# google-research/big_vision

Hardware: NVIDIA H100
Metric: siglip_vit_b16_pairs_per_sec (higher is better)
Workload: dtype bf16

## Files before the change

big_vision_b200/csrc/api.cu:

```cuda
#include "../../include/bv_b200.h"

#include "host_utils.h"
#include "kernels.h"

using namespace bv;

static inline cudaStream_t S(void* s) { return reinterpret_cast<cudaStream_t>(s); }

extern "C" {

const char* bv_last_error_string(void) { return last_error(); }
int bv_version(void) { return 100; }

int bv_device_supported(void) {
  int dev = 0;
  if (cudaGetDevice(&dev) != cudaSuccess) return 0;
  int major = 0;
  if (cudaDeviceGetAttribute(&major, cudaDevAttrComputeCapabilityMajor, dev) != cudaSuccess) return 0;
  return major == 9 ? 1 : 0;
}

int bv_gemm(const bv_gemm_args* a, void* stream) {
  if (!a) { set_error("bv_gemm: null args"); return BV_ERR_INVALID; }
  GemmArgs g;
  g.A = a->A; g.B = a->B; g.D = a->D; g.D2 = a->D2; g.bias = a->bias; g.aux = a->aux;
  g.colsum = a->colsum;
  g.M = a->M; g.N = a->N; g.K = a->K;
  g.lda = a->lda; g.ldb = a->ldb; g.ldd = a->ldd; g.ldd2 = a->ldd2; g.ldaux = a->ldaux;
  g.a_mn = a->a_mn; g.b_mn = a->b_mn; g.epi = a->epilogue; g.out_dtype = a->out_dtype;
  g.reduce_out = a->reduce_out; g.splits = a->splits; g.block_n = a->block_n;
  g.aux_row_mod = a->aux_row_mod; g.alpha = a->alpha;
  return launch_gemm(g, S(stream));
}

int bv_layernorm_fwd(const void* x, int x_dtype, const float* scale, const float* bias, void* y,
                     int y_dtype, float* mean, float* rstd, int64_t rows, int32_t d, float eps,
                     void* stream) {
  return launch_layernorm_fwd(x, x_dtype, scale, bias, y, y_dtype, mean, rstd, rows, d, eps, S(stream));
}
int bv_layernorm_bwd(const void* dy, int dy_dtype, const void* x, int x_dtype, const float* scale,
                     const float* mean, const float* rstd, const void* dres, void* dx,
                     int dx_dtype, float* dscale, float* dbias, float* dx_colsum, int64_t rows,
                     int32_t d, void* stream) {
  return launch_layernorm_bwd(dy, dy_dtype, x, x_dtype, scale, mean, rstd, dres, dx, dx_dtype,
                              dscale, dbias, dx_colsum, rows, d, S(stream));
}

static AttnArgs to_attn(const bv_attn_args& a) {
  AttnArgs r;
  r.q = a.q; r.k = a.k; r.v = a.v; r.o = a.o; r.lse = a.lse;
  r.B = a.B; r.H = a.H; r.Nq = a.Nq; r.Nk = a.Nk;
  r.ldq = a.ldq; r.ldk = a.ldk; r.ldv = a.ldv; r.ldo = a.ldo;
  r.bsq = a.bsq; r.bsk = a.bsk; r.bsv = a.bsv; r.bso = a.bso;
  r.scale = a.scale;
  return r;
}
int bv_attention_fwd(const bv_attn_args* a, void* stream) { return bv_attention_fwd_hd(a, 64, stream); }
int bv_attention_fwd_hd(const bv_attn_args* a, int32_t head_dim, void* stream) {
  if (!a) { set_error("bv_attention_fwd: null args"); return BV_ERR_INVALID; }
  return launch_attention_fwd(to_attn(*a), head_dim, S(stream));
}
int bv_attention_bwd(const bv_attn_bwd_args* a, void* stream) { return bv_attention_bwd_hd(a, 64, stream); }
int bv_attention_bwd_hd(const bv_attn_bwd_args* a, int32_t head_dim, void* stream) {
  if (!a) { set_error("bv_attention_bwd: null args"); return BV_ERR_INVALID; }
  AttnBwdArgs g;
  g.f = to_attn(a->fwd);
  g.d_o = a->d_o; g.lddo = a->lddo; g.bsdo = a->bsdo;
  g.dq = a->dq; g.dk = a->dk; g.dv = a->dv;
  g.lddq = a->lddq; g.lddk = a->lddk; g.lddv = a->lddv;
  g.bsdq = a->bsdq; g.bsdk = a->bsdk; g.bsdv = a->bsdv;
  g.dq_colsum = a->dq_colsum; g.dk_colsum = a->dk_colsum; g.dv_colsum = a->dv_colsum;
  g.delta = a->delta; g.dq_accum = a->dq_accum;
  return launch_attention_bwd(g, head_dim, S(stream));
}

int bv_patchify(const float* image, void* patches, int64_t n, int32_t H, int32_t W, int32_t C,
                int32_t P, void* stream) {
  return launch_patchify(image, patches, n, H, W, C, P, S(stream));
}
int bv_patchify_u8(const uint8_t* image, void* patches, int64_t n, int32_t H, int32_t W, int32_t C,
                   int32_t P, float vmin, float vmax, float in_min, float in_max, int32_t clip_values,
                   void* stream) {
  return launch_patchify_u8(image, patches, n, H, W, C, P, vmin, vmax, in_min, in_max, clip_values, S(stream));
}
int bv_embed_fwd(const int32_t* ids, const float* table, const float* pos, void* out,
                 int out_dtype, int64_t n, int32_t L, int32_t d, int32_t vocab, void* stream) {
  return launch_embed_fwd(ids, table, pos, out, out_dtype, n, L, d, vocab, S(stream));
}
int bv_embed_bwd(const int32_t* ids, const void* dy, int dy_dtype, float* dtable, float* dpos,
                 int64_t n, int32_t L, int32_t d, int32_t vocab, void* stream) {
  return launch_embed_bwd(ids, dy, dy_dtype, dtable, dpos, n, L, d, vocab, S(stream));
}
int bv_colsum(const void* x, int x_dtype, float* out, int64_t rows, int64_t cols, int64_t ld,
              void* stream) {
  return launch_colsum(x, x_dtype, out, rows, cols, ld, S(stream));
}
int bv_cast(const void* src, int src_dtype, void* dst, int dst_dtype, int64_t n, void* stream) {
  return launch_cast(src, src_dtype, dst, dst_dtype, n, S(stream));
}
int bv_l2norm_fwd(const void* x, int x_dtype, float* z, float* norm, int64_t n, int32_t d,
                  float eps, void* stream) {
  return launch_l2norm_fwd(x, x_dtype, z, norm, n, d, eps, S(stream));
}
int bv_l2norm_bwd(const float* dz, const float* z, const float* norm, void* dx, int dx_dtype,
                  int64_t n, int32_t d, float eps, void* stream) {
  return launch_l2norm_bwd(dz, z, norm, dx, dx_dtype, n, d, eps, S(stream));
}
int bv_pool_fwd(const void* x, int x_dtype, void* y, int y_dtype, int64_t n, int32_t N, int32_t d,
                int32_t mode, int32_t tok, void* stream) {
  return launch_pool(x, x_dtype, y, y_dtype, n, N, d, mode, tok, S(stream));
}
int bv_pool_bwd(const void* dy, int dy_dtype, void* dx, int dx_dtype, int64_t n, int32_t N,
                int32_t d, int32_t mode, int32_t tok, void* stream) {
  return launch_pool_bwd(dy, dy_dtype, dx, dx_dtype, n, N, d, mode, tok, S(stream));
}
int bv_pool_max_bwd(const void* dy, int dy_dtype, const void* x, int x_dtype, void* dx, int dx_dtype,
                    int64_t n, int32_t N, int32_t d, void* stream) {
  return launch_pool_max_bwd(dy, dy_dtype, x, x_dtype, dx, dx_dtype, n, N, d, S(stream));
}
int bv_broadcast_row(const void* x, int x_dtype, const float* row, void* y, int y_dtype,
                     int64_t rows, int32_t d, void* stream) {
  return launch_add_rows(x, x_dtype, row, y, y_dtype, rows, d, S(stream));
}
int bv_tanh_fwd(const void* x, void* y, int dtype, int64_t n, void* stream) {
  return launch_tanh_fwd(x, y, dtype, n, S(stream));
// ... 107 lines not shown
```

big_vision_b200/csrc/attention.cu:

```cuda
#include "common.cuh"
#include "host_utils.h"
#include "kernels.h"

namespace bv {

namespace {

constexpr int T = 64;
constexpr int BOX_BYTES = T * 64 * 2;
constexpr float LOG2E = 1.4426950408889634f;
constexpr float LN2 = 0.6931471805599453f;
constexpr int THREADS = 128;

template <int DH>
struct Geo {
  static_assert(DH == 64 || DH == 72 || DH == 80 || DH == 96 || DH == 104, "head dims 64, 72, 80, 96, 104");
  static constexpr int TILE_BYTES = DH > 64 ? 2 * BOX_BYTES : BOX_BYTES;
  static constexpr int KSTEPS = (DH + 15) / 16;
  static_assert(KSTEPS >= 4 && KSTEPS <= 8, "one or two 64-column boxes");
  static constexpr int R = DH / 2;
  static constexpr int FWD_SMEM = 5 * TILE_BYTES + 1024 + 64;
  static constexpr int BWD_SMEM = 6 * TILE_BYTES + BOX_BYTES + 1024 + 64;
};

__device__ __forceinline__ float ex2(float x) {
  float y;
  asm("ex2.approx.ftz.f32 %0, %1;" : "=f"(y) : "f"(x));
  return y;
}

int make_tmap_bnd(CUtensorMap* m, const void* ptr, int dh, int H, int64_t N, int64_t B, int64_t ld, int64_t bs) {
  if (dh == 64) {
    uint64_t dims[3] = {static_cast<uint64_t>(H) * 64, static_cast<uint64_t>(N), static_cast<uint64_t>(B)};
    uint64_t strides[2] = {static_cast<uint64_t>(ld) * 2, static_cast<uint64_t>(bs) * 2};
    uint32_t box[3] = {64, T, 1};
    return make_tmap(m, CU_TENSOR_MAP_DATA_TYPE_BFLOAT16, 3, ptr, dims, strides, box, true);
  }
  uint64_t dims[4] = {static_cast<uint64_t>(dh), static_cast<uint64_t>(H), static_cast<uint64_t>(N),
                      static_cast<uint64_t>(B)};
  uint64_t strides[3] = {static_cast<uint64_t>(dh) * 2, static_cast<uint64_t>(ld) * 2, static_cast<uint64_t>(bs) * 2};
  uint32_t box[4] = {64, 1, T, 1};
  return make_tmap(m, CU_TENSOR_MAP_DATA_TYPE_BFLOAT16, 4, ptr, dims, strides, box, true);
}

template <int DH>
__device__ __forceinline__ void load_tile(uint32_t dst, const CUtensorMap* m, uint32_t bar, int h, int row, int b) {
  if constexpr (DH == 64) {
    tma_load_3d(dst, m, bar, h * DH, row, b);
  } else {
    tma_load_4d(dst, m, bar, 0, h, row, b);
    tma_load_4d(dst + BOX_BYTES, m, bar, 64, h, row, b);
  }
}

__device__ __forceinline__ uint64_t desc_k(uint32_t tile) { return wgmma_desc_sw128(tile, 16u, 1024u); }
__device__ __forceinline__ uint64_t desc_mn(uint32_t tile) { return wgmma_desc_sw128(tile, 8192u, 1024u); }
constexpr uint64_t KSTEP_K = 32 >> 4, KSTEP_MN = 2048 >> 4;

template <int TA, int TB, int R>
__device__ __forceinline__ void wgmma_ss_dh(float (&d)[R], uint64_t a, uint64_t b, int scale_d) {
  if constexpr (R == 32) wgmma_ss_n64<TA, TB>(d, a, b, scale_d);
  else if constexpr (R == 36) wgmma_ss_n72<TA, TB>(d, a, b, scale_d);
  else if constexpr (R == 40) wgmma_ss_n80<TA, TB>(d, a, b, scale_d);
  else if constexpr (R == 48) wgmma_ss_n96<TA, TB>(d, a, b, scale_d);
  else wgmma_ss_n104<TA, TB>(d, a, b, scale_d);
}
template <int TB, int R>
__device__ __forceinline__ void wgmma_rs_dh(float (&d)[R], const uint32_t (&a)[4], uint64_t b, int scale_d) {
  if constexpr (R == 32) wgmma_rs_n64<TB>(d, a, b, scale_d);
  else if constexpr (R == 36) wgmma_rs_n72<TB>(d, a, b, scale_d);
  else if constexpr (R == 40) wgmma_rs_n80<TB>(d, a, b, scale_d);
  else if constexpr (R == 48) wgmma_rs_n96<TB>(d, a, b, scale_d);
  else wgmma_rs_n104<TB>(d, a, b, scale_d);
}

template <int DH>
__device__ __forceinline__ void mma_tile_kk(float (&d)[32], uint32_t a_tile, uint32_t b_tile) {
  const uint64_t a = desc_k(a_tile), b = desc_k(b_tile);
#pragma unroll
  for (int k = 0; k < 4; ++k) wgmma_ss_n64<0, 0>(d, a + k * KSTEP_K, b + k * KSTEP_K, k > 0 ? 1 : 0);
  if constexpr (DH > 64) {
    const uint64_t a1 = desc_k(a_tile + BOX_BYTES), b1 = desc_k(b_tile + BOX_BYTES);
#pragma unroll
    for (int k = 0; k < Geo<DH>::KSTEPS - 4; ++k) wgmma_ss_n64<0, 0>(d, a1 + k * KSTEP_K, b1 + k * KSTEP_K, 1);
  }
}
template <int R>
__device__ __forceinline__ void mma_tile_rs(float (&d)[R], const uint32_t (&p)[4][4], uint32_t b_tile) {
  const uint64_t b = desc_mn(b_tile);
#pragma unroll
  for (int k = 0; k < 4; ++k) wgmma_rs_dh<1>(d, p[k], b + k * KSTEP_MN, 1);
}

__device__ __forceinline__ void to_frags(const float (&s)[32], uint32_t (&p)[4][4]) {
#pragma unroll
  for (int kk = 0; kk < 4; ++kk) {
    p[kk][0] = pack_bf16(s[8 * kk + 0], s[8 * kk + 1]);
    p[kk][1] = pack_bf16(s[8 * kk + 2], s[8 * kk + 3]);
    p[kk][2] = pack_bf16(s[8 * kk + 4], s[8 * kk + 5]);
    p[kk][3] = pack_bf16(s[8 * kk + 6], s[8 * kk + 7]);
  }
}

template <int R>
__device__ __forceinline__ void zero(float (&d)[R]) {
#pragma unroll
  for (int i = 0; i < R; ++i) d[i] = 0.f;
}

struct FwdDev {
  int H, Nq, Nk, QT, NB;
  float scale_log2;
  float* lse;
  bf16* o;
  long long ldo, bso;
};

template <int DH>
__global__ void __launch_bounds__(THREADS)
// ... 48 lines not shown
      const int key = kbase + 8 * (i >> 2) + (i & 1);
      s[i] = key < p.Nk ? s[i] * p.scale_log2 : -INFINITY;
      mx[(i >> 1) & 1] = fmaxf(mx[(i >> 1) & 1], s[i]);
    }
    float corr[2];
#pragma unroll
    for (int r = 0; r < 2; ++r) {
      mx[r] = fmaxf(mx[r], __shfl_xor_sync(0xffffffffu, mx[r], 1));
      mx[r] = fmaxf(mx[r], __shfl_xor_sync(0xffffffffu, mx[r], 2));
      corr[r] = ex2(m[r] - mx[r]);
      m[r] = mx[r];
      l[r] *= corr[r];
    }
#pragma unroll
    for (int i = 0; i < 32; ++i) {
      const int r = (i >> 1) & 1;
      s[i] = ex2(s[i] - m[r]);
      l[r] += s[i];
      o[i] *= corr[r];
    }
#pragma unroll
    for (int i = 32; i < G::R; ++i) o[i] *= corr[(i >> 1) & 1];
    uint32_t pf[4][4];
    to_frags(s, pf);
    wgmma_fence_regs(o);
    wgmma_fence();
    mma_tile_rs(o, pf, v_s + slot * TILE_BYTES);
    wgmma_commit();
    wgmma_wait<0>();
    wgmma_fence_regs(o);
    __syncthreads();
    if (tid == 0 && j + 2 < p.NB) load_kv(j + 2);
  }
#pragma unroll
  for (int r = 0; r < 2; ++r) {
    l[r] += __shfl_xor_sync(0xffffffffu, l[r], 1);
    l[r] += __shfl_xor_sync(0xffffffffu, l[r], 2);
  }
  const float inv[2] = {1.f / l[0], 1.f / l[1]};
#pragma unroll
  for (int r = 0; r < 2; ++r) {
    const int q = qt * T + 16 * warp + (lane >> 2) + 8 * r;
    if (q >= p.Nq) continue;
    bf16* orow = p.o + b * p.bso + static_cast<long long>(q) * p.ldo + h * DH + 2 * (lane & 3);
#pragma unroll
    for (int jj = 0; jj < DH / 8; ++jj)
      *reinterpret_cast<uint32_t*>(orow + 8 * jj) = pack_bf16(o[4 * jj + 2 * r] * inv[r], o[4 * jj + 2 * r + 1] * inv[r]);
    if ((lane & 3) == 0) p.lse[(static_cast<long long>(b) * p.H + h) * p.Nq + q] = (m[r] + __log2f(l[r])) * LN2;
  }
}

struct BwdDev {
  int H, Nq, Nk, QT, KT;
  long long B;
  float scale, scale_log2;
  const float* lse;
  const float* delta;
  float* dq_accum;
  bf16* dk; bf16* dv;
  long long lddk, bsdk, lddv, bsdv;
  float* dk_colsum; float* dv_colsum;
};

template <int R>
__device__ __forceinline__ void tile_colsum(const float (&d)[R], float mul, int row0, int nvalid, float* colsum,
                                            int lane) {
#pragma unroll
  for (int jj = 0; jj < R / 4; ++jj) {
    float c[2] = {0.f, 0.f};
#pragma unroll
    for (int r = 0; r < 2; ++r) {
      if (row0 + 8 * r >= nvalid) continue;
      c[0] += round_bf16(d[4 * jj + 2 * r] * mul);
      c[1] += round_bf16(d[4 * jj + 2 * r + 1] * mul);
    }
#pragma unroll
    for (int e = 0; e < 2; ++e) {
      c[e] += __shfl_xor_sync(0xffffffffu, c[e], 4);
      c[e] += __shfl_xor_sync(0xffffffffu, c[e], 8);
      c[e] += __shfl_xor_sync(0xffffffffu, c[e], 16);
    }
    if (lane < 4) {
      atomicAdd(colsum + 8 * jj + 2 * lane, c[0]);
      atomicAdd(colsum + 8 * jj + 2 * lane + 1, c[1]);
    }
  }
}

template <int DH>
__global__ void __launch_bounds__(THREADS)
attn_bwd_kernel(const __grid_constant__ CUtensorMap tmQ, const __grid_constant__ CUtensorMap tmK,
                const __grid_constant__ CUtensorMap tmV, const __grid_constant__ CUtensorMap tmdO, const BwdDev p) {
  using G = Geo<DH>;
  constexpr int TILE_BYTES = G::TILE_BYTES;
  extern __shared__ uint8_t smem_raw[];
  const uint32_t k_s = (smem_u32(smem_raw) + 1023u) & ~1023u, v_s = k_s + TILE_BYTES, q_s = k_s + 2 * TILE_BYTES,
                 do_s = k_s + 4 * TILE_BYTES, ds_s = k_s + 6 * TILE_BYTES;
  const uint32_t kv_bar = ds_s + BOX_BYTES;
  auto q_bar = [&](int s) { return kv_bar + 8u * (1 + s); };

  const int kt = static_cast<int>(blockIdx.x % p.KT);
  const int bh = static_cast<int>(blockIdx.x / p.KT);
  const int h = bh % p.H, b = bh / p.H;
  const int tid = threadIdx.x, lane = tid & 31, warp = tid >> 5;

  auto load_q = [&](int i) {
    const int s = i & 1;
    mbar_expect_tx(q_bar(s), 2 * TILE_BYTES);
    load_tile<DH>(q_s + s * TILE_BYTES, &tmQ, q_bar(s), h, i * T, b);
    load_tile<DH>(do_s + s * TILE_BYTES, &tmdO, q_bar(s), h, i * T, b);
  };
  if (tid == 0) {
    mbar_init(kv_bar, 1);
    mbar_init(q_bar(0), 1);
    mbar_init(q_bar(1), 1);
    fence_barrier_init();
    mbar_expect_tx(kv_bar, 2 * TILE_BYTES);
    load_tile<DH>(k_s, &tmK, kv_bar, h, kt * T, b);
    load_tile<DH>(v_s, &tmV, kv_bar, h, kt * T, b);
    load_q(0);
    if (p.QT > 1) load_q(1);
  }
  __syncthreads();

  float dk[G::R], dv[G::R];
  zero(dk);
  zero(dv);
  const long long bhq = (static_cast<long long>(b) * p.H + h) * p.Nq;
  const int cols = p.H * DH;
  const int key_row = 16 * warp + (lane >> 2);
  mbar_wait(kv_bar, 0);
  for (int i = 0; i < p.QT; ++i) {
    const int slot = i & 1;
    mbar_wait(q_bar(slot), (i >> 1) & 1);
    const uint32_t qi = q_s + slot * TILE_BYTES, doi = do_s + slot * TILE_BYTES;
    float st[32], dpt[32];
    wgmma_fence();
    mma_tile_kk<DH>(st, k_s, qi);
    mma_tile_kk<DH>(dpt, v_s, doi);
    wgmma_commit();
    float lse2[16], dl[16];
#pragma unroll
    for (int c = 0; c < 16; ++c) {
      const int q = i * T + 8 * (c >> 1) + 2 * (lane & 3) + (c & 1);
      lse2[c] = q < p.Nq ? p.lse[bhq + q] * LOG2E : INFINITY;
      dl[c] = q < p.Nq ? p.delta[bhq + q] : 0.f;
    }
    wgmma_wait<0>();
    wgmma_fence_regs(st);
    wgmma_fence_regs(dpt);
#pragma unroll
    for (int e = 0; e < 32; ++e) {
      const int c = 2 * (e >> 2) + (e & 1);
      st[e] = ex2(st[e] * p.scale_log2 - lse2[c]);
      dpt[e] = st[e] * (dpt[e] - dl[c]);
    }
    uint32_t pf[4][4], sf[4][4];
    to_frags(st, pf);
    to_frags(dpt, sf);
#pragma unroll
    for (int kk = 0; kk < 4; ++kk) {
#pragma unroll
      for (int f = 0; f < 4; ++f) {
        const int r = key_row + 8 * (f & 1);
        const int chunk = 2 * kk + (f >> 1);
        const uint32_t addr = ds_s + r * 128 + ((chunk ^ (r & 7)) << 4) + 4 * (lane & 3);
        asm volatile("st.shared.b32 [%0], %1;" ::"r"(addr), "r"(sf[kk][f]) : "memory");
      }
    }
    fence_proxy_async();
    __syncthreads();
    float dq[G::R];
    wgmma_fence_regs(dv);
    wgmma_fence_regs(dk);
    wgmma_fence();
    mma_tile_rs(dv, pf, doi);
    mma_tile_rs(dk, sf, qi);
    {
      const uint64_t a = desc_mn(ds_s), bk = desc_mn(k_s);
#pragma unroll
      for (int k = 0; k < 4; ++k) wgmma_ss_dh<1, 1>(dq, a + k * KSTEP_MN, bk + k * KSTEP_MN, k > 0 ? 1 : 0);
    }
    wgmma_commit();
    wgmma_wait<0>();
    wgmma_fence_regs(dv);
    wgmma_fence_regs(dk);
    wgmma_fence_regs(dq);
#pragma unroll
    for (int r = 0; r < 2; ++r) {
      const int q = i * T + 16 * warp + (lane >> 2) + 8 * r;
      if (q >= p.Nq) continue;
      float* dst = p.dq_accum + ((static_cast<long long>(kt) * p.B + b) * p.Nq + q) * cols + h * DH + 2 * (lane & 3);
#pragma unroll
      for (int jj = 0; jj < DH / 8; ++jj)
        *reinterpret_cast<float2*>(dst + 8 * jj) = make_float2(dq[4 * jj + 2 * r] * p.scale,
                                                               dq[4 * jj + 2 * r + 1] * p.scale);
    }
    __syncthreads();
    if (tid == 0 && i + 2 < p.QT) load_q(i + 2);
  }
  const int k0 = kt * T + key_row;
#pragma unroll
  for (int r = 0; r < 2; ++r) {
    const int key = k0 + 8 * r;
    if (key >= p.Nk) continue;
    bf16* kr = p.dk + b * p.bsdk + static_cast<long long>(key) * p.lddk + h * DH + 2 * (lane & 3);
    bf16* vr = p.dv + b * p.bsdv + static_cast<long long>(key) * p.lddv + h * DH + 2 * (lane & 3);
#pragma unroll
    for (int jj = 0; jj < DH / 8; ++jj) {
      *reinterpret_cast<uint32_t*>(kr + 8 * jj) = pack_bf16(dk[4 * jj + 2 * r] * p.scale, dk[4 * jj + 2 * r + 1] * p.scale);
      *reinterpret_cast<uint32_t*>(vr + 8 * jj) = pack_bf16(dv[4 * jj + 2 * r], dv[4 * jj + 2 * r + 1]);
    }
  }
  if (p.dk_colsum != nullptr) tile_colsum(dk, p.scale, k0, p.Nk, p.dk_colsum + h * DH, lane);
  if (p.dv_colsum != nullptr) tile_colsum(dv, 1.f, k0, p.Nk, p.dv_colsum + h * DH, lane);
}

template <int DH>
__global__ void __launch_bounds__(256)
attn_delta_kernel(const bf16* __restrict__ o, const bf16* __restrict__ d_o, float* __restrict__ delta,
                  int64_t B, int H, int N, int64_t ldo, int64_t bso, int64_t lddo, int64_t bsdo) {
  constexpr int LOG2_LANES = DH == 64 ? 3 : 4, LANES = 1 << LOG2_LANES;
  const int64_t total = B * N * H;
  const int chunk = threadIdx.x & (LANES - 1);
  for (int64_t r = (blockIdx.x * static_cast<int64_t>(blockDim.x) + threadIdx.x) >> LOG2_LANES; r < total;
       r += (static_cast<int64_t>(gridDim.x) * blockDim.x) >> LOG2_LANES) {
    const int h = static_cast<int>(r % H);
    const int64_t bt = r / H;
    const int t = static_cast<int>(bt % N);
    const int64_t b = bt / N;
    float acc = 0.f;
    if (chunk < DH / 8) {
      const uint4 ao = ld_nc_na(reinterpret_cast<const uint4*>(o + b * bso + t * ldo + h * DH + chunk * 8));
      const uint4 ad = ld_nc_na(reinterpret_cast<const uint4*>(d_o + b * bsdo + t * lddo + h * DH + chunk * 8));
      acc = bf16_lo(ao.x) * bf16_lo(ad.x) + bf16_hi(ao.x) * bf16_hi(ad.x);
      acc += bf16_lo(ao.y) * bf16_lo(ad.y) + bf16_hi(ao.y) * bf16_hi(ad.y);
      acc += bf16_lo(ao.z) * bf16_lo(ad.z) + bf16_hi(ao.z) * bf16_hi(ad.z);
      acc += bf16_lo(ao.w) * bf16_lo(ad.w) + bf16_hi(ao.w) * bf16_hi(ad.w);
    }
#pragma unroll
    for (int off = 1; off < LANES; off <<= 1) acc += __shfl_xor_sync(0xffffffffu, acc, off);
    if (chunk == 0) delta[(b * H + h) * N + t] = acc;
  }
}

__global__ void __launch_bounds__(256)
attn_dq_convert_kernel(const float* __restrict__ acc, int KT, bf16* __restrict__ dq, float* __restrict__ colsum,
                       int64_t rows_total, int N, int cols, int64_t lddq, int64_t bsdq, int rows_per_block) {
  const int groups = cols / 8;
  const int rlanes = 256 / groups > 0 ? 256 / groups : 1;
  const int cg = threadIdx.x % groups, rl = threadIdx.x / groups;
  const int64_t r0 = static_cast<int64_t>(blockIdx.x) * rows_per_block;
  float cs[8] = {0.f, 0.f, 0.f, 0.f, 0.f, 0.f, 0.f, 0.f};
  if (rl < rlanes) {
    for (int64_t r = r0 + rl; r < r0 + rows_per_block && r < rows_total; r += rlanes) {
      float4 a = *reinterpret_cast<const float4*>(acc + r * cols + cg * 8);
      float4 c = *reinterpret_cast<const float4*>(acc + r * cols + cg * 8 + 4);
      for (int kt = 1; kt < KT; ++kt) {
        const float* src = acc + (kt * rows_total + r) * cols + cg * 8;
        const float4 a2 = *reinterpret_cast<const float4*>(src), c2 = *reinterpret_cast<const float4*>(src + 4);
        a.x += a2.x; a.y += a2.y; a.z += a2.z; a.w += a2.w;
        c.x += c2.x; c.y += c2.y; c.z += c2.z; c.w += c2.w;
      }
      uint4 q;
      q.x = pack_bf16(a.x, a.y); q.y = pack_bf16(a.z, a.w);
      q.z = pack_bf16(c.x, c.y); q.w = pack_bf16(c.z, c.w);
      const int64_t b = r / N;
      const int t = static_cast<int>(r % N);
      *reinterpret_cast<uint4*>(dq + b * bsdq + t * lddq + cg * 8) = q;
      cs[0] += bf16_lo(q.x); cs[1] += bf16_hi(q.x); cs[2] += bf16_lo(q.y); cs[3] += bf16_hi(q.y);
      cs[4] += bf16_lo(q.z); cs[5] += bf16_hi(q.z); cs[6] += bf16_lo(q.w); cs[7] += bf16_hi(q.w);
    }
    if (colsum != nullptr) {
#pragma unroll
      for (int k = 0; k < 8; ++k) atomicAdd(colsum + cg * 8 + k, cs[k]);
    }
  }
}

int check_head_dim(int head_dim, const char* who) {
  if (head_dim == 64 || head_dim == 72 || head_dim == 80 || head_dim == 96 || head_dim == 104) return BV_OK;
  set_error("%s: head_dim %d is not supported (supported head dims: 64, 72, 80, 96, 104)", who, head_dim);
  return BV_ERR_UNSUPPORTED;
}

int check_attn(const AttnArgs& a, const char* who) {
  if (a.B <= 0 || a.H <= 0 || a.Nq <= 0 || a.Nk <= 0 || a.Nq > 65536 || a.Nk > 65536) {
    set_error("%s: need 1 <= Nq,Nk <= 65536 and B,H >= 1 (got B=%lld H=%d Nq=%d Nk=%d)", who,
              (long long)a.B, a.H, a.Nq, a.Nk);
    return BV_ERR_INVALID;
  }
  const int64_t tiles = ((a.Nq > a.Nk ? a.Nq : a.Nk) + T - 1) / T;
  if (a.B * a.H * tiles > 0x7fffffffLL) {
    set_error("%s: too many (batch, head, tile) work units", who);
    return BV_ERR_INVALID;
  }
  if ((reinterpret_cast<uintptr_t>(a.o) & 15) || (a.ldo % 8) || (a.bso % 8)) {
    set_error("%s: o must be 16B aligned with strides that are multiples of 8", who);
    return BV_ERR_INVALID;
  }
  return BV_OK;
}

template <int DH>
int attention_fwd(const AttnArgs& a, cudaStream_t s) {
  using G = Geo<DH>;
  int rc = check_attn(a, "bv_attention_fwd");
  if (rc) return rc;
  FwdDev p;
  p.H = a.H; p.Nq = a.Nq; p.Nk = a.Nk;
  p.QT = (a.Nq + T - 1) / T;
  p.NB = (a.Nk + T - 1) / T;
  p.scale_log2 = a.scale * LOG2E;
  p.lse = a.lse;
  p.o = static_cast<bf16*>(a.o);
  p.ldo = a.ldo; p.bso = a.bso;
  CUtensorMap tmQ, tmK, tmV;
  if ((rc = make_tmap_bnd(&tmQ, a.q, DH, a.H, a.Nq, a.B, a.ldq, a.bsq))) return rc;
  if ((rc = make_tmap_bnd(&tmK, a.k, DH, a.H, a.Nk, a.B, a.ldk, a.bsk))) return rc;
  if ((rc = make_tmap_bnd(&tmV, a.v, DH, a.H, a.Nk, a.B, a.ldv, a.bsv))) return rc;
  const long long grid = a.B * a.H * p.QT;
  rc = check_cuda(cudaFuncSetAttribute(attn_fwd_kernel<DH>, cudaFuncAttributeMaxDynamicSharedMemorySize, G::FWD_SMEM),
                  "cudaFuncSetAttribute(attn_fwd)");
  if (rc) return rc;
  attn_fwd_kernel<DH><<<static_cast<unsigned>(grid), THREADS, G::FWD_SMEM, s>>>(tmQ, tmK, tmV, p);
  return check_cuda(cudaGetLastError(), "attn_fwd_kernel launch");
}

template <int DH>
int attention_bwd(const AttnBwdArgs& g, cudaStream_t s) {
  using G = Geo<DH>;
  const AttnArgs& a = g.f;
  int rc = check_attn(a, "bv_attention_bwd");
  if (rc) return rc;
  if (a.lse == nullptr) { set_error("bv_attention_bwd: lse required"); return BV_ERR_INVALID; }
  if (g.dq_accum == nullptr || g.delta == nullptr) {
    set_error("bv_attention_bwd: needs the dq_accum [ceil(Nk/64),B,Nq,H*head_dim] and delta [B,H,Nq] fp32 workspaces");
    return BV_ERR_INVALID;
  }
  if ((reinterpret_cast<uintptr_t>(g.d_o) & 15) || (g.lddo % 8) || (g.bsdo % 8)) {
    set_error("bv_attention_bwd: d_o must be 16B aligned with strides that are multiples of 8");
    return BV_ERR_INVALID;
  }
  const void* grads[3] = {g.dq, g.dk, g.dv};
  const int64_t lds[3] = {g.lddq, g.lddk, g.lddv}, bss[3] = {g.bsdq, g.bsdk, g.bsdv};
  for (int i = 0; i < 3; ++i) {
    if (grads[i] == nullptr || (reinterpret_cast<uintptr_t>(grads[i]) & 15) || (lds[i] % 8) || (bss[i] % 8)) {
      set_error("bv_attention_bwd: dq / dk / dv must be non-null, 16B aligned, with strides that are multiples of 8");
      return BV_ERR_INVALID;
    }
  }
  if (a.H * DH > 2048) { set_error("bv_attention_bwd: H*head_dim must be <= 2048"); return BV_ERR_INVALID; }
  const int cols = a.H * DH;
  {
    constexpr int lanes = DH == 64 ? 8 : 16;
    const int64_t head_rows = a.B * a.Nq * a.H;
    int64_t blocks = (head_rows * lanes + 255) / 256;
    const int64_t cap = static_cast<int64_t>(num_sms()) * 16;
    if (blocks > cap) blocks = cap;
    attn_delta_kernel<DH><<<static_cast<unsigned>(blocks), 256, 0, s>>>(
        reinterpret_cast<const bf16*>(a.o), reinterpret_cast<const bf16*>(g.d_o), g.delta, a.B, a.H, a.Nq,
        a.ldo, a.bso, g.lddo, g.bsdo);
    if ((rc = check_cuda(cudaGetLastError(), "attn_delta_kernel launch"))) return rc;
  }
  BwdDev p;
  p.H = a.H; p.Nq = a.Nq; p.Nk = a.Nk; p.B = a.B;
  p.QT = (a.Nq + T - 1) / T;
  p.KT = (a.Nk + T - 1) / T;
  p.scale = a.scale;
  p.scale_log2 = a.scale * LOG2E;
  p.lse = a.lse;
  p.delta = g.delta;
  p.dq_accum = g.dq_accum;
  p.dk = static_cast<bf16*>(g.dk); p.dv = static_cast<bf16*>(g.dv);
  p.lddk = g.lddk; p.bsdk = g.bsdk; p.lddv = g.lddv; p.bsdv = g.bsdv;
  p.dk_colsum = g.dk_colsum; p.dv_colsum = g.dv_colsum;
  CUtensorMap tmQ, tmK, tmV, tmdO;
  if ((rc = make_tmap_bnd(&tmQ, a.q, DH, a.H, a.Nq, a.B, a.ldq, a.bsq))) return rc;
  if ((rc = make_tmap_bnd(&tmK, a.k, DH, a.H, a.Nk, a.B, a.ldk, a.bsk))) return rc;
  if ((rc = make_tmap_bnd(&tmV, a.v, DH, a.H, a.Nk, a.B, a.ldv, a.bsv))) return rc;
  if ((rc = make_tmap_bnd(&tmdO, g.d_o, DH, a.H, a.Nq, a.B, g.lddo, g.bsdo))) return rc;
  const long long grid = a.B * a.H * p.KT;
  rc = check_cuda(cudaFuncSetAttribute(attn_bwd_kernel<DH>, cudaFuncAttributeMaxDynamicSharedMemorySize, G::BWD_SMEM),
                  "cudaFuncSetAttribute(attn_bwd)");
  if (rc) return rc;
  attn_bwd_kernel<DH><<<static_cast<unsigned>(grid), THREADS, G::BWD_SMEM, s>>>(tmQ, tmK, tmV, tmdO, p);
  if ((rc = check_cuda(cudaGetLastError(), "attn_bwd_kernel launch"))) return rc;
  {
    const int64_t rows = a.B * a.Nq;
    const int rows_per_block = 256;
    const int64_t blocks = (rows + rows_per_block - 1) / rows_per_block;
    attn_dq_convert_kernel<<<static_cast<unsigned>(blocks), 256, 0, s>>>(
        g.dq_accum, p.KT, reinterpret_cast<bf16*>(g.dq), g.dq_colsum, rows, a.Nq, cols, g.lddq, g.bsdq,
        rows_per_block);
    rc = check_cuda(cudaGetLastError(), "attn_dq_convert_kernel launch");
  }
  return rc;
}

}

int launch_attention_fwd(const AttnArgs& a, int head_dim, cudaStream_t s) {
  int rc = check_head_dim(head_dim, "bv_attention_fwd");
  if (rc) return rc;
  switch (head_dim) {
    case 72: return attention_fwd<72>(a, s);
    case 80: return attention_fwd<80>(a, s);
    case 96: return attention_fwd<96>(a, s);
    case 104: return attention_fwd<104>(a, s);
    default: return attention_fwd<64>(a, s);
  }
}

int launch_attention_bwd(const AttnBwdArgs& g, int head_dim, cudaStream_t s) {
  int rc = check_head_dim(head_dim, "bv_attention_bwd");
  if (rc) return rc;
  switch (head_dim) {
    case 72: return attention_bwd<72>(g, s);
    case 80: return attention_bwd<80>(g, s);
    case 96: return attention_bwd<96>(g, s);
    case 104: return attention_bwd<104>(g, s);
    default: return attention_bwd<64>(g, s);
  }
}

}
```

big_vision_b200/csrc/kernels.h:

```cpp
#pragma once
#include <cuda_runtime.h>
#include <stdint.h>

namespace bv {

enum : int { EPI_NONE = 0, EPI_BIAS = 1, EPI_BIAS_GELU = 2, EPI_BIAS_RESID = 3, EPI_DGELU = 4,
             EPI_BIAS_GELU_ACT = 5 };

struct GemmArgs {
  const void* A; const void* B; void* D; void* D2;
  const float* bias; const void* aux;
  float* colsum;
  int64_t M, N, K;
  int64_t lda, ldb, ldd, ldd2, ldaux;
  int a_mn, b_mn;
  int epi, out_dtype, reduce_out, splits, block_n, aux_row_mod;
  float alpha;
};
int launch_gemm(const GemmArgs& g, cudaStream_t stream);

int launch_layernorm_fwd(const void* x, int x_dtype, const float* scale, const float* bias,
                         void* y, int y_dtype, float* mean, float* rstd, int64_t rows, int d,
                         float eps, cudaStream_t s);
int launch_layernorm_bwd(const void* dy, int dy_dtype, const void* x, int x_dtype,
                         const float* scale, const float* mean, const float* rstd,
                         const void* dres, void* dx, int dx_dtype, float* dscale, float* dbias,
                         float* dres_colsum, int64_t rows, int d, cudaStream_t s);

struct AttnArgs {
  const void* q; const void* k; const void* v;
  void* o;
  float* lse;
  int64_t B; int H; int Nq; int Nk;
  int64_t ldq, ldk, ldv, ldo;
  int64_t bsq, bsk, bsv, bso;
  float scale;
};
int launch_attention_fwd(const AttnArgs& a, int head_dim, cudaStream_t s);
struct AttnBwdArgs {
  AttnArgs f;
  const void* d_o; int64_t lddo, bsdo;
  void* dq; void* dk; void* dv;
  float* dq_colsum; float* dk_colsum; float* dv_colsum;
  int64_t lddq, lddk, lddv, bsdq, bsdk, bsdv;
  float* delta;
  float* dq_accum;
};
int launch_attention_bwd(const AttnBwdArgs& a, int head_dim, cudaStream_t s);

int launch_top1(const void* logits, int dtype, int64_t rows, int C, int64_t ld, int32_t* idx,
                const float* labels, int64_t ldl, const float* mask, float* top1_correct,
                float* sums, cudaStream_t s);
int launch_retrieval_ranks(const float* dist, int64_t NI, int64_t NT, int64_t ld, const int32_t* corr,
                           int32_t* rank_t2i, int32_t* rank_i2t, cudaStream_t s);

int launch_patchify(const float* img, void* out, int64_t n, int H, int W, int C, int P,
                    cudaStream_t s);
int launch_patchify_u8(const uint8_t* img, void* out, int64_t n, int H, int W, int C, int P, float vmin,
                       float vmax, float in_min, float in_max, int clip, cudaStream_t s);
int launch_untranspose_add(const void* y, const void* res, void* out, int64_t n, int N, int d,
                           cudaStream_t s);
int launch_concat_cls(const void* x, const float* cls, void* out, int64_t n, int N0, int d,
                      cudaStream_t s);
int launch_drop_cls(const void* x, void* out, int64_t n, int N0, int d, cudaStream_t s);
int launch_embed_fwd(const int32_t* ids, const float* table, const float* pos, void* out,
                     int out_dtype, int64_t n, int L, int d, int vocab, cudaStream_t s);
int launch_embed_bwd(const int32_t* ids, const void* dy, int dy_dtype, float* dtable, float* dpos,
                     int64_t n, int L, int d, int vocab, cudaStream_t s);
int launch_colsum(const void* x, int x_dtype, float* out, int64_t rows, int64_t cols, int64_t ld,
                  cudaStream_t s);
int launch_cast(const void* src, int src_dtype, void* dst, int dst_dtype, int64_t n,
                cudaStream_t s);
int launch_l2norm_fwd(const void* x, int x_dtype, float* z, float* norm, int64_t n, int d,
                      float eps, cudaStream_t s);
int launch_l2norm_bwd(const float* dz, const float* z, const float* norm, void* dx, int dx_dtype,
                      int64_t n, int d, float eps, cudaStream_t s);
int launch_pool(const void* x, int x_dtype, void* y, int y_dtype, int64_t n, int N, int d,
                int mode, int tok_offset, cudaStream_t s);
int launch_pool_bwd(const void* dy, int dy_dtype, void* dx, int dx_dtype, int64_t n, int N, int d,
                    int mode, int tok_offset, cudaStream_t s);
int launch_pool_max_bwd(const void* dy, int dy_dtype, const void* x, int x_dtype, void* dx,
                        int dx_dtype, int64_t n, int N, int d, cudaStream_t s);
int launch_add_rows(const void* x, int x_dtype, const float* row, void* y, int y_dtype,
                    int64_t rows, int d, cudaStream_t s);
int launch_tanh_fwd(const void* x, void* y, int dtype, int64_t n, cudaStream_t s);
int launch_tanh_bwd(const void* dy, const void* y, void* dx, int dtype, int64_t n, cudaStream_t s);
int launch_gelu_fwd(const void* x, void* y, int dtype, int64_t n, cudaStream_t s);
int launch_mixup(const float* x, float* out, int64_t n, int64_t row_elems, float a, cudaStream_t s);
int launch_axpby(const void* x, const void* y, void* out, int dtype, float a, float b, int64_t n,
                 cudaStream_t s);
int launch_transpose_tokens(const void* x, void* y, int64_t n, int N, int d, cudaStream_t s);
int launch_row_select(const void* a, const void* b, const float* mask, void* out, int64_t n, int N,
                      int d, cudaStream_t s);

int launch_siglip_loss_ew(const float* dots, int64_t n, int64_t B, int64_t ld, int64_t row_offset,
                          const float* t_param, const float* b_param, int64_t global_B, void* G,
                          int64_t ldg, float* loss, float* dt, float* db, float* partials,
                          cudaStream_t s);
int launch_softmax_contrastive(const float* dots, int64_t n, int64_t B, int64_t ld, int64_t row_offset,
// ... 35 lines not shown
```

big_vision_b200/ops.py:

```python
import ctypes
import math

import torch

from big_vision_b200 import lib as L

_DT = {torch.float32: L.F32, torch.bfloat16: L.BF16}


def _dt(t):
  try:
    return _DT[t.dtype]
  except KeyError:
    raise L.BvError(f"unsupported dtype {t.dtype}") from None


def _p(t):
  if t is None:
    return None
  if not t.is_cuda:
    raise L.BvError("bv_b200 kernels need CUDA tensors (no CPU fallback)")
  return ctypes.c_void_p(t.data_ptr())


# ... 78 lines not shown
  return dx


def _attn_view(t):
  assert t.dim() == 3 and t.stride(2) == 1, (t.shape, t.stride())
  return t.data_ptr(), t.stride(1), t.stride(0)


def _attn_args(q, k, v, o, lse, heads, scale):
  B, Nq, _ = q.shape
  Nk = k.shape[1]
  qp, ldq, bsq = _attn_view(q)
  kp, ldk, bsk = _attn_view(k)
  vp, ldv, bsv = _attn_view(v)
  op, ldo, bso = _attn_view(o)
  return L.AttnArgs(q=qp, k=kp, v=vp, o=op, lse=lse.data_ptr(), B=B, H=heads, Nq=Nq, Nk=Nk,
                    ldq=ldq, ldk=ldk, ldv=ldv, ldo=ldo, bsq=bsq, bsk=bsk, bsv=bsv, bso=bso,
                    scale=scale)


ATTN_HEAD_DIMS = (64, 72, 80, 96, 104)


def _head_dim(cols, heads):
  if cols % heads:
    raise ValueError(f"attention: {cols} columns do not split into {heads} heads")
  return cols // heads


def attention_fwd(q, k, v, heads, scale=None):
  B, Nq, cols = q.shape
  dh = _head_dim(cols, heads)
  if scale is None:
    scale = 1.0 / math.sqrt(dh)
  o = torch.empty((B, Nq, cols), dtype=torch.bfloat16, device=q.device)
  lse = torch.empty((B, heads, Nq), dtype=torch.float32, device=q.device)
  args = _attn_args(q, k, v, o, lse, heads, scale)
  L.call("bv_attention_fwd_hd", ctypes.byref(args), dh, _stream())
  return o, lse


def attention_bwd(do, q, k, v, o, lse, heads, scale=None, dq=None, dk=None, dv=None,
                  dq_colsum=None, dk_colsum=None, dv_colsum=None):
  dh = _head_dim(q.shape[2], heads)
  if scale is None:
    scale = 1.0 / math.sqrt(dh)
  if dq is None:
    dq = torch.empty(q.shape, dtype=torch.bfloat16, device=q.device)
  if dk is None:
    dk = torch.empty(k.shape, dtype=torch.bfloat16, device=q.device)
  if dv is None:
    dv = torch.empty(v.shape, dtype=torch.bfloat16, device=q.device)
  f = _attn_args(q, k, v, o, lse, heads, scale)
  B, Nq, cols = q.shape
  delta = torch.empty((B, heads, Nq), dtype=torch.float32, device=q.device)
  dq_accum = torch.empty(((k.shape[1] + 63) // 64, B, Nq, cols), dtype=torch.float32, device=q.device)
  dop, lddo, bsdo = _attn_view(do)
  dqp, lddq, bsdq = _attn_view(dq)
  dkp, lddk, bsdk = _attn_view(dk)
  dvp, lddv, bsdv = _attn_view(dv)
  args = L.AttnBwdArgs(fwd=f, d_o=dop, lddo=lddo, bsdo=bsdo, dq=dqp, dk=dkp, dv=dvp,
                       lddq=lddq, lddk=lddk, lddv=lddv, bsdq=bsdq, bsdk=bsdk, bsdv=bsdv,
                       dq_colsum=dq_colsum.data_ptr() if dq_colsum is not None else None,
                       dk_colsum=dk_colsum.data_ptr() if dk_colsum is not None else None,
                       dv_colsum=dv_colsum.data_ptr() if dv_colsum is not None else None,
                       delta=delta.data_ptr(), dq_accum=dq_accum.data_ptr())
  L.call("bv_attention_bwd_hd", ctypes.byref(args), dh, _stream())
  L.LAUNCHES[0] += 2
  return dq, dk, dv


def patchify(image, patch, value_range=(-1.0, 1.0), in_range=(0.0, 255.0), clip_values=False):
  n, H, W, C = image.shape
  assert image.is_contiguous()
  if image.dtype == torch.uint8:
    kp = (patch * patch * C + 7) // 8 * 8
    out = torch.empty((n * (H // patch) * (W // patch), kp), dtype=torch.bfloat16, device=image.device)
    L.call("bv_patchify_u8", _p(image), _p(out), n, H, W, C, patch, float(value_range[0]),
           float(value_range[1]), float(in_range[0]), float(in_range[1]), int(clip_values), _stream())
    return out
  assert image.dtype == torch.float32
  kp = (patch * patch * C + 7) // 8 * 8
  out = torch.empty((n * (H // patch) * (W // patch), kp), dtype=torch.bfloat16, device=image.device)
  L.call("bv_patchify", _p(image), _p(out), n, H, W, C, patch, _stream())
  return out


def embed_fwd(ids, table, pos, out_dtype=torch.bfloat16):
  n, Ln = ids.shape
  vocab, d = table.shape
  assert ids.dtype == torch.int32 and ids.is_contiguous()
  out = torch.empty((n * Ln, d), dtype=out_dtype, device=table.device)
  L.call("bv_embed_fwd", _p(ids), _p(table), _p(pos), _p(out), _dt(out), n, Ln, d, vocab, _stream())
  return out


def embed_bwd(ids, dy, dtable, dpos):
  n, Ln = ids.shape
  vocab, d = dtable.shape
  L.call("bv_embed_bwd", _p(ids), _p(dy), _dt(dy), _p(dtable), _p(dpos), n, Ln, d, vocab, _stream())


def colsum(x, out):
  x, ld = _rowmajor(x)
  L.call("bv_colsum", _p(x), _dt(x), _p(out), x.shape[0], x.shape[1], ld, _stream())
  return out


def cast(src, dst):
  assert src.is_contiguous() and dst.is_contiguous() and src.numel() == dst.numel()
  L.call("bv_cast", _p(src), _dt(src), _p(dst), _dt(dst), src.numel(), _stream())
  return dst


def l2norm_fwd(x, eps=1e-8):
  n, d = x.shape
  z = torch.empty((n, d), dtype=torch.float32, device=x.device)
  norm = torch.empty((n,), dtype=torch.float32, device=x.device)
  L.call("bv_l2norm_fwd", _p(x), _dt(x), _p(z), _p(norm), n, d, eps, _stream())
# ... 214 lines not shown
```

Baseline: 2705.

## Split attention backward into separate dQ and dK/dV kernels, dropping fp32 dQ accumulation

Attention backward is split into two kernels. A new per-query-tile kernel recomputes S and dP over all key tiles and writes dQ in bf16 directly, applying the column sum itself. The dK/dV kernel no longer stages dS in shared memory, no longer computes per-key-tile dQ partials, and no longer writes them to a large fp32 workspace. This removes that workspace, its global memory traffic and the separate reduce/convert kernel. The cost is recomputing the QK^T and dO·V^T matmuls and the softmax in the dQ kernel.

```diff
diff --git a/big_vision_b200/csrc/api.cu b/big_vision_b200/csrc/api.cu
--- a/big_vision_b200/csrc/api.cu
+++ b/big_vision_b200/csrc/api.cu
@@ -70,7 +70,7 @@
   g.lddq = a->lddq; g.lddk = a->lddk; g.lddv = a->lddv;
   g.bsdq = a->bsdq; g.bsdk = a->bsdk; g.bsdv = a->bsdv;
   g.dq_colsum = a->dq_colsum; g.dk_colsum = a->dk_colsum; g.dv_colsum = a->dv_colsum;
-  g.delta = a->delta; g.dq_accum = a->dq_accum;
+  g.delta = a->delta;
   return launch_attention_bwd(g, head_dim, S(stream));
 }
 
diff --git a/big_vision_b200/csrc/attention.cu b/big_vision_b200/csrc/attention.cu
--- a/big_vision_b200/csrc/attention.cu
+++ b/big_vision_b200/csrc/attention.cu
@@ -20,7 +20,7 @@
   static_assert(KSTEPS >= 4 && KSTEPS <= 8, "one or two 64-column boxes");
   static constexpr int R = DH / 2;
   static constexpr int FWD_SMEM = 5 * TILE_BYTES + 1024 + 64;
-  static constexpr int BWD_SMEM = 6 * TILE_BYTES + BOX_BYTES + 1024 + 64;
+  static constexpr int BWD_SMEM = 6 * TILE_BYTES + 1024 + 64;
 };
 
 __device__ __forceinline__ float ex2(float x) {
@@ -57,14 +57,6 @@
 __device__ __forceinline__ uint64_t desc_mn(uint32_t tile) { return wgmma_desc_sw128(tile, 8192u, 1024u); }
 constexpr uint64_t KSTEP_K = 32 >> 4, KSTEP_MN = 2048 >> 4;
 
-template <int TA, int TB, int R>
-__device__ __forceinline__ void wgmma_ss_dh(float (&d)[R], uint64_t a, uint64_t b, int scale_d) {
-  if constexpr (R == 32) wgmma_ss_n64<TA, TB>(d, a, b, scale_d);
-  else if constexpr (R == 36) wgmma_ss_n72<TA, TB>(d, a, b, scale_d);
-  else if constexpr (R == 40) wgmma_ss_n80<TA, TB>(d, a, b, scale_d);
-  else if constexpr (R == 48) wgmma_ss_n96<TA, TB>(d, a, b, scale_d);
-  else wgmma_ss_n104<TA, TB>(d, a, b, scale_d);
-}
 template <int TB, int R>
 __device__ __forceinline__ void wgmma_rs_dh(float (&d)[R], const uint32_t (&a)[4], uint64_t b, int scale_d) {
   if constexpr (R == 32) wgmma_rs_n64<TB>(d, a, b, scale_d);
@@ -219,14 +211,12 @@
 
 struct BwdDev {
   int H, Nq, Nk, QT, KT;
-  long long B;
   float scale, scale_log2;
   const float* lse;
   const float* delta;
-  float* dq_accum;
-  bf16* dk; bf16* dv;
-  long long lddk, bsdk, lddv, bsdv;
-  float* dk_colsum; float* dv_colsum;
+  bf16* dq; bf16* dk; bf16* dv;
+  long long lddq, bsdq, lddk, bsdk, lddv, bsdv;
+  float* dq_colsum; float* dk_colsum; float* dv_colsum;
 };
 
 template <int R>
@@ -256,14 +246,105 @@
 
 template <int DH>
 __global__ void __launch_bounds__(THREADS)
-attn_bwd_kernel(const __grid_constant__ CUtensorMap tmQ, const __grid_constant__ CUtensorMap tmK,
-                const __grid_constant__ CUtensorMap tmV, const __grid_constant__ CUtensorMap tmdO, const BwdDev p) {
+attn_bwd_dq_kernel(const __grid_constant__ CUtensorMap tmQ, const __grid_constant__ CUtensorMap tmK,
+                   const __grid_constant__ CUtensorMap tmV, const __grid_constant__ CUtensorMap tmdO, const BwdDev p) {
+  using G = Geo<DH>;
+  constexpr int TILE_BYTES = G::TILE_BYTES;
+  extern __shared__ uint8_t smem_raw[];
+  const uint32_t q_s = (smem_u32(smem_raw) + 1023u) & ~1023u, do_s = q_s + TILE_BYTES, k_s = q_s + 2 * TILE_BYTES,
+                 v_s = q_s + 4 * TILE_BYTES;
+  const uint32_t q_bar = q_s + 6 * TILE_BYTES;
+  auto kv_bar = [&](int s) { return q_bar + 8u * (1 + s); };
+
+  const int qt = static_cast<int>(blockIdx.x % p.QT);
+  const int bh = static_cast<int>(blockIdx.x / p.QT);
+  const int h = bh % p.H, b = bh / p.H;
+  const int tid = threadIdx.x, lane = tid & 31, warp = tid >> 5;
+
+  auto load_kv = [&](int j) {
+    const int s = j & 1;
+    mbar_expect_tx(kv_bar(s), 2 * TILE_BYTES);
+    load_tile<DH>(k_s + s * TILE_BYTES, &tmK, kv_bar(s), h, j * T, b);
+    load_tile<DH>(v_s + s * TILE_BYTES, &tmV, kv_bar(s), h, j * T, b);
+  };
+  if (tid == 0) {
+    mbar_init(q_bar, 1);
+    mbar_init(kv_bar(0), 1);
+    mbar_init(kv_bar(1), 1);
+    fence_barrier_init();
+    mbar_expect_tx(q_bar, 2 * TILE_BYTES);
+    load_tile<DH>(q_s, &tmQ, q_bar, h, qt * T, b);
+    load_tile<DH>(do_s, &tmdO, q_bar, h, qt * T, b);
+    load_kv(0);
+    if (p.KT > 1) load_kv(1);
+  }
+  __syncthreads();
+
+  float dq[G::R];
+  zero(dq);
+  const long long bhq = (static_cast<long long>(b) * p.H + h) * p.Nq;
+  const int q0 = qt * T + 16 * warp + (lane >> 2);
+  float lse2[2], dl[2];
+#pragma unroll
+  for (int r = 0; r < 2; ++r) {
+    const int q = q0 + 8 * r;
+    lse2[r] = q < p.Nq ? p.lse[bhq + q] * LOG2E : INFINITY;
+    dl[r] = q < p.Nq ? p.delta[bhq + q] : 0.f;
+  }
+  mbar_wait(q_bar, 0);
+  for (int j = 0; j < p.KT; ++j) {
+    const int slot = j & 1;
+    mbar_wait(kv_bar(slot), (j >> 1) & 1);
+    const uint32_t kj = k_s + slot * TILE_BYTES, vj = v_s + slot * TILE_BYTES;
+    float s[32], dp[32];
+    wgmma_fence();
+    mma_tile_kk<DH>(s, q_s, kj);
+    mma_tile_kk<DH>(dp, do_s, vj);
+    wgmma_commit();
+    wgmma_wait<0>();
+    wgmma_fence_regs(s);
+    wgmma_fence_regs(dp);
+    const int kbase = j * T + 2 * (lane & 3);
+#pragma unroll
+    for (int i = 0; i < 32; ++i) {
+      const int r = (i >> 1) & 1;
+      const int key = kbase + 8 * (i >> 2) + (i & 1);
+      const float pr = key < p.Nk ? ex2(s[i] * p.scale_log2 - lse2[r]) : 0.f;
+      dp[i] = pr * (dp[i] - dl[r]);
+    }
+    uint32_t sf[4][4];
+    to_frags(dp, sf);
+    wgmma_fence_regs(dq);
+    wgmma_fence();
+    mma_tile_rs(dq, sf, kj);
+    wgmma_commit();
+    wgmma_wait<0>();
+    wgmma_fence_regs(dq);
+    __syncthreads();
+    if (tid == 0 && j + 2 < p.KT) load_kv(j + 2);
+  }
+#pragma unroll
+  for (int r = 0; r < 2; ++r) {
+    const int q = q0 + 8 * r;
+    if (q >= p.Nq) continue;
+    bf16* qr = p.dq + b * p.bsdq + static_cast<long long>(q) * p.lddq + h * DH + 2 * (lane & 3);
+#pragma unroll
+    for (int jj = 0; jj < DH / 8; ++jj)
+      *reinterpret_cast<uint32_t*>(qr + 8 * jj) = pack_bf16(dq[4 * jj + 2 * r] * p.scale, dq[4 * jj + 2 * r + 1] * p.scale);
+  }
+  if (p.dq_colsum != nullptr) tile_colsum(dq, p.scale, q0, p.Nq, p.dq_colsum + h * DH, lane);
+}
+
+template <int DH>
+__global__ void __launch_bounds__(THREADS)
+attn_bwd_dkdv_kernel(const __grid_constant__ CUtensorMap tmQ, const __grid_constant__ CUtensorMap tmK,
+                     const __grid_constant__ CUtensorMap tmV, const __grid_constant__ CUtensorMap tmdO, const BwdDev p) {
   using G = Geo<DH>;
   constexpr int TILE_BYTES = G::TILE_BYTES;
   extern __shared__ uint8_t smem_raw[];
   const uint32_t k_s = (smem_u32(smem_raw) + 1023u) & ~1023u, v_s = k_s + TILE_BYTES, q_s = k_s + 2 * TILE_BYTES,
-                 do_s = k_s + 4 * TILE_BYTES, ds_s = k_s + 6 * TILE_BYTES;
-  const uint32_t kv_bar = ds_s + BOX_BYTES;
+                 do_s = k_s + 4 * TILE_BYTES;
+  const uint32_t kv_bar = k_s + 6 * TILE_BYTES;
   auto q_bar = [&](int s) { return kv_bar + 8u * (1 + s); };
 
   const int kt = static_cast<int>(blockIdx.x % p.KT);
@@ -294,7 +375,6 @@
   zero(dk);
   zero(dv);
   const long long bhq = (static_cast<long long>(b) * p.H + h) * p.Nq;
-  const int cols = p.H * DH;
   const int key_row = 16 * warp + (lane >> 2);
   mbar_wait(kv_bar, 0);
   for (int i = 0; i < p.QT; ++i) {
@@ -325,44 +405,15 @@
     uint32_t pf[4][4], sf[4][4];
     to_frags(st, pf);
     to_frags(dpt, sf);
-#pragma unroll
-    for (int kk = 0; kk < 4; ++kk) {
-#pragma unroll
-      for (int f = 0; f < 4; ++f) {
-        const int r = key_row + 8 * (f & 1);
-        const int chunk = 2 * kk + (f >> 1);
-        const uint32_t addr = ds_s + r * 128 + ((chunk ^ (r & 7)) << 4) + 4 * (lane & 3);
-        asm volatile("st.shared.b32 [%0], %1;" ::"r"(addr), "r"(sf[kk][f]) : "memory");
-      }
-    }
-    fence_proxy_async();
-    __syncthreads();
-    float dq[G::R];
     wgmma_fence_regs(dv);
     wgmma_fence_regs(dk);
     wgmma_fence();
     mma_tile_rs(dv, pf, doi);
     mma_tile_rs(dk, sf, qi);
-    {
-      const uint64_t a = desc_mn(ds_s), bk = desc_mn(k_s);
-#pragma unroll
-      for (int k = 0; k < 4; ++k) wgmma_ss_dh<1, 1>(dq, a + k * KSTEP_MN, bk + k * KSTEP_MN, k > 0 ? 1 : 0);
-    }
     wgmma_commit();
     wgmma_wait<0>();
     wgmma_fence_regs(dv);
     wgmma_fence_regs(dk);
-    wgmma_fence_regs(dq);
-#pragma unroll
-    for (int r = 0; r < 2; ++r) {
-      const int q = i * T + 16 * warp + (lane >> 2) + 8 * r;
-      if (q >= p.Nq) continue;
-      float* dst = p.dq_accum + ((static_cast<long long>(kt) * p.B + b) * p.Nq + q) * cols + h * DH + 2 * (lane & 3);
-#pragma unroll
-      for (int jj = 0; jj < DH / 8; ++jj)
-        *reinterpret_cast<float2*>(dst + 8 * jj) = make_float2(dq[4 * jj + 2 * r] * p.scale,
-                                                               dq[4 * jj + 2 * r + 1] * p.scale);
-    }
     __syncthreads();
     if (tid == 0 && i + 2 < p.QT) load_q(i + 2);
   }
@@ -408,40 +459,6 @@
 #pragma unroll
     for (int off = 1; off < LANES; off <<= 1) acc += __shfl_xor_sync(0xffffffffu, acc, off);
     if (chunk == 0) delta[(b * H + h) * N + t] = acc;
-  }
-}
-
-__global__ void __launch_bounds__(256)
-attn_dq_convert_kernel(const float* __restrict__ acc, int KT, bf16* __restrict__ dq, float* __restrict__ colsum,
-                       int64_t rows_total, int N, int cols, int64_t lddq, int64_t bsdq, int rows_per_block) {
-  const int groups = cols / 8;
-  const int rlanes = 256 / groups > 0 ? 256 / groups : 1;
-  const int cg = threadIdx.x % groups, rl = threadIdx.x / groups;
-  const int64_t r0 = static_cast<int64_t>(blockIdx.x) * rows_per_block;
-  float cs[8] = {0.f, 0.f, 0.f, 0.f, 0.f, 0.f, 0.f, 0.f};
-  if (rl < rlanes) {
-    for (int64_t r = r0 + rl; r < r0 + rows_per_block && r < rows_total; r += rlanes) {
-      float4 a = *reinterpret_cast<const float4*>(acc + r * cols + cg * 8);
-      float4 c = *reinterpret_cast<const float4*>(acc + r * cols + cg * 8 + 4);
-      for (int kt = 1; kt < KT; ++kt) {
-        const float* src = acc + (kt * rows_total + r) * cols + cg * 8;
-        const float4 a2 = *reinterpret_cast<const float4*>(src), c2 = *reinterpret_cast<const float4*>(src + 4);
-        a.x += a2.x; a.y += a2.y; a.z += a2.z; a.w += a2.w;
-        c.x += c2.x; c.y += c2.y; c.z += c2.z; c.w += c2.w;
-      }
-      uint4 q;
-      q.x = pack_bf16(a.x, a.y); q.y = pack_bf16(a.z, a.w);
-      q.z = pack_bf16(c.x, c.y); q.w = pack_bf16(c.z, c.w);
-      const int64_t b = r / N;
-      const int t = static_cast<int>(r % N);
-      *reinterpret_cast<uint4*>(dq + b * bsdq + t * lddq + cg * 8) = q;
-      cs[0] += bf16_lo(q.x); cs[1] += bf16_hi(q.x); cs[2] += bf16_lo(q.y); cs[3] += bf16_hi(q.y);
-      cs[4] += bf16_lo(q.z); cs[5] += bf16_hi(q.z); cs[6] += bf16_lo(q.w); cs[7] += bf16_hi(q.w);
-    }
-    if (colsum != nullptr) {
-#pragma unroll
-      for (int k = 0; k < 8; ++k) atomicAdd(colsum + cg * 8 + k, cs[k]);
-    }
   }
 }
 
@@ -501,8 +518,8 @@
   int rc = check_attn(a, "bv_attention_bwd");
   if (rc) return rc;
   if (a.lse == nullptr) { set_error("bv_attention_bwd: lse required"); return BV_ERR_INVALID; }
-  if (g.dq_accum == nullptr || g.delta == nullptr) {
-    set_error("bv_attention_bwd: needs the dq_accum [ceil(Nk/64),B,Nq,H*head_dim] and delta [B,H,Nq] fp32 workspaces");
+  if (g.delta == nullptr) {
+    set_error("bv_attention_bwd: needs the delta [B,H,Nq] fp32 workspace");
     return BV_ERR_INVALID;
   }
   if ((reinterpret_cast<uintptr_t>(g.d_o) & 15) || (g.lddo % 8) || (g.bsdo % 8)) {
@@ -517,8 +534,6 @@
       return BV_ERR_INVALID;
     }
   }
-  if (a.H * DH > 2048) { set_error("bv_attention_bwd: H*head_dim must be <= 2048"); return BV_ERR_INVALID; }
-  const int cols = a.H * DH;
   {
     constexpr int lanes = DH == 64 ? 8 : 16;
     const int64_t head_rows = a.B * a.Nq * a.H;
@@ -531,37 +546,31 @@
     if ((rc = check_cuda(cudaGetLastError(), "attn_delta_kernel launch"))) return rc;
   }
   BwdDev p;
-  p.H = a.H; p.Nq = a.Nq; p.Nk = a.Nk; p.B = a.B;
+  p.H = a.H; p.Nq = a.Nq; p.Nk = a.Nk;
   p.QT = (a.Nq + T - 1) / T;
   p.KT = (a.Nk + T - 1) / T;
   p.scale = a.scale;
   p.scale_log2 = a.scale * LOG2E;
   p.lse = a.lse;
   p.delta = g.delta;
-  p.dq_accum = g.dq_accum;
-  p.dk = static_cast<bf16*>(g.dk); p.dv = static_cast<bf16*>(g.dv);
-  p.lddk = g.lddk; p.bsdk = g.bsdk; p.lddv = g.lddv; p.bsdv = g.bsdv;
-  p.dk_colsum = g.dk_colsum; p.dv_colsum = g.dv_colsum;
+  p.dq = static_cast<bf16*>(g.dq); p.dk = static_cast<bf16*>(g.dk); p.dv = static_cast<bf16*>(g.dv);
+  p.lddq = g.lddq; p.bsdq = g.bsdq; p.lddk = g.lddk; p.bsdk = g.bsdk; p.lddv = g.lddv; p.bsdv = g.bsdv;
+  p.dq_colsum = g.dq_colsum; p.dk_colsum = g.dk_colsum; p.dv_colsum = g.dv_colsum;
   CUtensorMap tmQ, tmK, tmV, tmdO;
   if ((rc = make_tmap_bnd(&tmQ, a.q, DH, a.H, a.Nq, a.B, a.ldq, a.bsq))) return rc;
   if ((rc = make_tmap_bnd(&tmK, a.k, DH, a.H, a.Nk, a.B, a.ldk, a.bsk))) return rc;
   if ((rc = make_tmap_bnd(&tmV, a.v, DH, a.H, a.Nk, a.B, a.ldv, a.bsv))) return rc;
   if ((rc = make_tmap_bnd(&tmdO, g.d_o, DH, a.H, a.Nq, a.B, g.lddo, g.bsdo))) return rc;
-  const long long grid = a.B * a.H * p.KT;
-  rc = check_cuda(cudaFuncSetAttribute(attn_bwd_kernel<DH>, cudaFuncAttributeMaxDynamicSharedMemorySize, G::BWD_SMEM),
-                  "cudaFuncSetAttribute(attn_bwd)");
+  rc = check_cuda(cudaFuncSetAttribute(attn_bwd_dq_kernel<DH>, cudaFuncAttributeMaxDynamicSharedMemorySize, G::BWD_SMEM),
+                  "cudaFuncSetAttribute(attn_bwd_dq)");
   if (rc) return rc;
-  attn_bwd_kernel<DH><<<static_cast<unsigned>(grid), THREADS, G::BWD_SMEM, s>>>(tmQ, tmK, tmV, tmdO, p);
-  if ((rc = check_cuda(cudaGetLastError(), "attn_bwd_kernel launch"))) return rc;
-  {
-    const int64_t rows = a.B * a.Nq;
-    const int rows_per_block = 256;
-    const int64_t blocks = (rows + rows_per_block - 1) / rows_per_block;
-    attn_dq_convert_kernel<<<static_cast<unsigned>(blocks), 256, 0, s>>>(
-        g.dq_accum, p.KT, reinterpret_cast<bf16*>(g.dq), g.dq_colsum, rows, a.Nq, cols, g.lddq, g.bsdq,
-        rows_per_block);
-    rc = check_cuda(cudaGetLastError(), "attn_dq_convert_kernel launch");
-  }
+  attn_bwd_dq_kernel<DH><<<static_cast<unsigned>(a.B * a.H * p.QT), THREADS, G::BWD_SMEM, s>>>(tmQ, tmK, tmV, tmdO, p);
+  if ((rc = check_cuda(cudaGetLastError(), "attn_bwd_dq_kernel launch"))) return rc;
+  rc = check_cuda(cudaFuncSetAttribute(attn_bwd_dkdv_kernel<DH>, cudaFuncAttributeMaxDynamicSharedMemorySize, G::BWD_SMEM),
+                  "cudaFuncSetAttribute(attn_bwd_dkdv)");
+  if (rc) return rc;
+  attn_bwd_dkdv_kernel<DH><<<static_cast<unsigned>(a.B * a.H * p.KT), THREADS, G::BWD_SMEM, s>>>(tmQ, tmK, tmV, tmdO, p);
+  rc = check_cuda(cudaGetLastError(), "attn_bwd_dkdv_kernel launch");
   return rc;
 }
 
diff --git a/big_vision_b200/csrc/kernels.h b/big_vision_b200/csrc/kernels.h
--- a/big_vision_b200/csrc/kernels.h
+++ b/big_vision_b200/csrc/kernels.h
@@ -44,7 +44,6 @@
   float* dq_colsum; float* dk_colsum; float* dv_colsum;
   int64_t lddq, lddk, lddv, bsdq, bsdk, bsdv;
   float* delta;
-  float* dq_accum;
 };
 int launch_attention_bwd(const AttnBwdArgs& a, int head_dim, cudaStream_t s);
 
diff --git a/big_vision_b200/ops.py b/big_vision_b200/ops.py
--- a/big_vision_b200/ops.py
+++ b/big_vision_b200/ops.py
@@ -154,9 +154,8 @@
   if dv is None:
     dv = torch.empty(v.shape, dtype=torch.bfloat16, device=q.device)
   f = _attn_args(q, k, v, o, lse, heads, scale)
-  B, Nq, cols = q.shape
+  B, Nq, _ = q.shape
   delta = torch.empty((B, heads, Nq), dtype=torch.float32, device=q.device)
-  dq_accum = torch.empty(((k.shape[1] + 63) // 64, B, Nq, cols), dtype=torch.float32, device=q.device)
   dop, lddo, bsdo = _attn_view(do)
   dqp, lddq, bsdq = _attn_view(dq)
   dkp, lddk, bsdk = _attn_view(dk)
@@ -166,7 +165,7 @@
                        dq_colsum=dq_colsum.data_ptr() if dq_colsum is not None else None,
                        dk_colsum=dk_colsum.data_ptr() if dk_colsum is not None else None,
                        dv_colsum=dv_colsum.data_ptr() if dv_colsum is not None else None,
-                       delta=delta.data_ptr(), dq_accum=dq_accum.data_ptr())
+                       delta=delta.data_ptr())
   L.call("bv_attention_bwd_hd", ctypes.byref(args), dh, _stream())
   L.LAUNCHES[0] += 2
   return dq, dk, dv
```

Result: faster. 2821, median of 6 (+4.3%).
